# yumingj/Text2Human

Hardware: AMD Instinct MI355X
Metric: 512x256 images/sec (sample_from_parsing) (higher is better)
Workload: dtype f16 hi plane + e4m3 cross-term planes, f32 accumulate (hidden err 4e-5, tokens exact); exact-f32: exact_fp32_path

## Files before the change

### text2human_amd/csrc/gemm_split.hip

```cpp
#include <hip/hip_ext.h>
#include <stdlib.h>

#include <type_traits>

#include "common.h"

namespace {

typedef t2h_f16x8 f16x8;
typedef unsigned int u32x4 __attribute__((ext_vector_type(4)));

constexpr int SP_TILE_B = T2H_SPLIT_TILE_B;
constexpr int SP_LDS_ROW = 144;
constexpr int SP_PIECES = 8;

__device__ __forceinline__ void gload16_async(u32x4& dst, const char* ptr) {
#ifdef T2H_SDBG_NOGLOAD
  asm volatile("" : "=v"(dst) : "v"(ptr));
#else
  asm volatile("global_load_dwordx4 %0, %1, off" : "=v"(dst) : "v"(ptr) : "memory");
#endif
}
__device__ __forceinline__ void gload16_async(u32x4& dst, unsigned voff, const char* sbase) {
#ifdef T2H_SDBG_NOGLOAD
  asm volatile("" : "=v"(dst) : "v"(voff), "s"(sbase));
#else
  asm volatile("global_load_dwordx4 %0, %1, %2" : "=v"(dst) : "v"(voff), "s"(sbase) : "memory");
#endif
}
template <int N>
__device__ __forceinline__ void wait_vmcnt16(u32x4& v) {
  asm volatile("s_waitcnt vmcnt(%1)" : "+v"(v) : "n"(N));
}

__device__ __forceinline__ float erf_rational(float x) {
  x = fminf(fmaxf(x, -4.0f), 4.0f);
  const float x2 = x * x;
  float p = -2.72614225801306e-10f;
  p = fmaf(p, x2, 2.77068142495902e-08f);
  p = fmaf(p, x2, -2.10102402082508e-06f);
  p = fmaf(p, x2, -5.69250639462346e-05f);
  p = fmaf(p, x2, -7.34990630326855e-04f);
  p = fmaf(p, x2, -2.95459980854025e-03f);
  p = fmaf(p, x2, -1.60960333262415e-02f);
  float q = -1.45660718464996e-05f;
  q = fmaf(q, x2, -2.13374055278905e-04f);
  q = fmaf(q, x2, -1.68282697438203e-03f);
  q = fmaf(q, x2, -7.37332916720468e-03f);
  q = fmaf(q, x2, -1.42647390514189e-02f);
  return x * p * __builtin_amdgcn_rcpf(q);
}

__device__ __forceinline__ float gelu_erf_s(float v) {
  return 0.5f * v * (1.0f + erf_rational(v * 0.70710678118654752440f));
}

typedef float f32x2 __attribute__((ext_vector_type(2)));
__device__ __forceinline__ f32x2 gelu_erf_2(f32x2 v) {
  f32x2 x = v * 0.70710678118654752440f;
  x[0] = fminf(fmaxf(x[0], -4.0f), 4.0f);
  x[1] = fminf(fmaxf(x[1], -4.0f), 4.0f);
  const f32x2 x2 = x * x;
  auto fma2 = [](f32x2 a, f32x2 b, float c) { return __builtin_elementwise_fma(a, b, f32x2{c, c}); };
  f32x2 p = {-2.72614225801306e-10f, -2.72614225801306e-10f};
  p = fma2(p, x2, 2.77068142495902e-08f);
  p = fma2(p, x2, -2.10102402082508e-06f);
  p = fma2(p, x2, -5.69250639462346e-05f);
  p = fma2(p, x2, -7.34990630326855e-04f);
  p = fma2(p, x2, -2.95459980854025e-03f);
  p = fma2(p, x2, -1.60960333262415e-02f);
  f32x2 q = {-1.45660718464996e-05f, -1.45660718464996e-05f};
  q = fma2(q, x2, -2.13374055278905e-04f);
  q = fma2(q, x2, -1.68282697438203e-03f);
  q = fma2(q, x2, -7.37332916720468e-03f);
  q = fma2(q, x2, -1.42647390514189e-02f);
  const f32x2 rq = {__builtin_amdgcn_rcpf(q[0]), __builtin_amdgcn_rcpf(q[1])};
  const f32x2 e = x * p * rq;
  return (v * 0.5f) * (e + 1.0f);
}
__device__ __forceinline__ f32x4 gelu_erf_v(f32x4 v) {
  const f32x2 a = gelu_erf_2(f32x2{v[0], v[1]}), b = gelu_erf_2(f32x2{v[2], v[3]});
  return f32x4{a[0], a[1], b[0], b[1]};
}

#ifdef T2H_SDBG_HOTLOAD
#define LM0 0
#define LN0 0
#else
#define LM0 m0
#define LN0 n0
#endif

#define G1_MARK(i)                                                                                      \
  do {                                                                                                  \
    if (probe != nullptr && threadIdx.x == 0) {                                                         \
      probe[(int64_t)blockIdx.x * 16 + (i)] = (long long)__builtin_amdgcn_s_memrealtime();              \
      probe[(int64_t)blockIdx.x * 16 + 8 + (i)] = (long long)__builtin_amdgcn_s_memtime();              \
    }                                                                                                   \
  } while (0)

typedef int i32x8 __attribute__((ext_vector_type(8)));
__device__ __forceinline__ f32x16 x8_cross(const f16x8& a0, const f16x8& a1, const f16x8& b0, const f16x8& b1, const f32x16& c) {
  union { f16x8 h[2]; i32x8 v; } ua, ub;
  ua.h[0] = a0;
  ua.h[1] = a1;
  ub.h[0] = b0;
  ub.h[1] = b1;
  return __builtin_amdgcn_mfma_scale_f32_32x32x64_f8f6f4(ua.v, ub.v, c, 0, 0, 0, 0x7f7f7f7f, 0, 0x7f7f7f7f);
}

template <int BM, int BN, int WARPS_M, int WARPS_N, int KS, int PP, int FMT = 0>
__global__ __launch_bounds__(64 * WARPS_M * WARPS_N * KS) void gemm_split_kernel(const t2h_gemm_split_args p, int* const ovf, long long* const probe) {
  constexpr int NT = 64 * WARPS_M * WARPS_N;
  constexpr int NWG = WARPS_M * WARPS_N;
  constexpr int WM = BM / WARPS_M, WN = BN / WARPS_N;
  constexpr int TM = WM / 32, TN = WN / 32;
  static_assert(TM >= 1 && TN >= 1, "wave tile must hold a 32x32 MFMA tile");
  constexpr int PIECES = (BM + BN) * SP_PIECES;
  constexpr int L = (PIECES + NT - 1) / NT;
  constexpr int NMMA = 2 * 3 * TM * TN;
  constexpr int BUF_B = (BM + BN) * SP_LDS_ROW;
  constexpr int O_LD = WN + 4;
  constexpr int OT_LD = WM + 4;
  constexpr int OW = WM * O_LD > WN * OT_LD ? WM * O_LD : WN * OT_LD;
  constexpr int EPI_B = OW * 4 * NWG * KS;
  constexpr int TILE_IMG_B = (BM + BN) * SP_TILE_B;
  constexpr int MAIN_B = PP == 2 ? 3 * TILE_IMG_B : 2 * BUF_B * KS;
  constexpr int SMEM_B = MAIN_B > EPI_B ? MAIN_B : EPI_B;

  __shared__ __attribute__((aligned(16))) char smem[SMEM_B];

  G1_MARK(0);
  const int kg = KS == 1 ? 0 : (int)threadIdx.x / NT;
  const int tid = threadIdx.x - kg * NT;
  const int lane = tid & 63, wave = tid >> 6;
  char* const gsm = smem + kg * (2 * BUF_B);
  const int l31 = lane & 31, hh = lane >> 5;
  const int wm0 = (wave / WARPS_N) * WM, wn0 = (wave % WARPS_N) * WN;
  const int nbx = (p.N + BN - 1) / BN, nby = (p.M + BM - 1) / BM;
  const int ksid = (PP == 2 && p.ksplit > 1) ? __builtin_amdgcn_readfirstlane((int)blockIdx.x / (nbx * nby)) : 0;
  int m0, n0;
  {
    const int total = nbx * nby, b = (int)blockIdx.x - ksid * (nbx * nby);
    const int xcd = b & 7, slot = b >> 3, q = total >> 3, r = total & 7;
    const int lin = (xcd < r ? xcd * (q + 1) : r * (q + 1) + (xcd - r) * q) + slot;
    int mt = lin / nbx, nt = lin - mt * nbx;
    if (r == 0 && q <= 32 && nbx >= 16 && (nbx & 1) == 0 && (nby & 3) == 0 && q == (nby >> 2) * (nbx >> 1)) {
      const int hbx = nbx >> 1;
      const int sr = slot / hbx;
      mt = (xcd >> 1) * (nby >> 2) + sr;
      nt = (xcd & 1) * hbx + (slot - sr * hbx);
    }
    m0 = mt * BM;
    n0 = nt * BN;
  }
  const int nk_row = p.K / (32 * KS);
  const int nk = (PP == 2 && p.ksplit > 1) ? nk_row >> (p.ksplit >> 1) : nk_row;
  const int last = nk - 1;
  const int64_t row_b = (int64_t)nk_row * (SP_TILE_B * KS);
  const int64_t k_base = (int64_t)__builtin_amdgcn_readfirstlane(ksid * nk) * SP_TILE_B;
  constexpr int K_STEP_B = SP_TILE_B * KS;

  f32x16 acc[2][TM][TN];
#pragma unroll
  for (int c = 0; c < 2; ++c)
#pragma unroll
    for (int i = 0; i < TM; ++i)
#pragma unroll
      for (int j = 0; j < TN; ++j)
#pragma unroll
        for (int r = 0; r < 16; ++r) acc[c][i][j][r] = 0.f;

  if constexpr (PP == 2) {
    static_assert(KS == 1 && NWG == 8 && (BM + BN) % 64 == 0, "ping-pong DMA: 8 waves, whole 8-row groups per wave");
    constexpr int NL = (BM + BN) / 64;
    const int grp = __builtin_amdgcn_readfirstlane(wave >> 2);
    auto pp_barrier = [] {
      __builtin_amdgcn_sched_barrier(0);
#ifndef T2H_SDBG_NOBAR
      __builtin_amdgcn_s_barrier();
#endif
      __builtin_amdgcn_sched_barrier(0);
    };
    const unsigned lds0 = (unsigned)(uintptr_t)smem;
    unsigned goff[NL];
#pragma unroll
    for (int i = 0; i < NL; ++i) {
      const int g = wave + 8 * i;
      const int r = g * 8 + (lane >> 3), pc = (lane & 7) ^ ((r >> 1) & 7);
      const bool isA = r < BM;
      const int grow = isA ? min(LM0 + r, p.M - 1) : min(LN0 + r - BM, p.N - 1);
      goff[i] = (unsigned)grow * (unsigned)row_b + pc * 16;
    }
    static_assert(BM % 64 == 0, "an 8-row group belongs to one operand");
    const unsigned wdst = __builtin_amdgcn_readfirstlane(lds0 + wave * 1024);
    auto dma = [&](int kt, unsigned buf_off) {
      if (kt > last) return;
      const int64_t k0 = (int64_t)kt * SP_TILE_B + k_base;
      const char* const baseA = reinterpret_cast<const char*>(p.A) + k0;
      const char* const baseB = reinterpret_cast<const char*>(p.B) + k0;
#pragma unroll
      for (int i = 0; i < NL; ++i) {
#ifndef T2H_SDBG_NOGLOAD
        unsigned keep;
#ifdef T2H_SDBG_HALFDMA
        if (i & 1) continue;
#endif
        const char* const base = i < BM / 64 ? baseA : baseB;
        const unsigned dst_i = wdst + buf_off + i * 8192;
#ifndef T2H_DMA_POLICY
#define T2H_DMA_POLICY " nt"
#endif
        asm volatile("s_mov_b32 %0, m0\n\ts_mov_b32 m0, %3\n\ts_nop 0\n\tglobal_load_lds_dwordx4 %1, %2" T2H_DMA_POLICY "\n\ts_mov_b32 m0, %0"
                     : "=&s"(keep)
                     : "v"(goff[i]), "s"(base), "s"(dst_i)
                     : "memory");
#endif
      }
    };
    auto wait_landed = [&](bool younger_in_flight) {
      __builtin_amdgcn_sched_barrier(0);
      if (younger_in_flight) asm volatile("s_waitcnt vmcnt(%0)" ::"n"(NL) : "memory");
      else asm volatile("s_waitcnt vmcnt(0)" ::: "memory");
      __builtin_amdgcn_sched_barrier(0);
    };
    const int swz = (l31 >> 1) & 7;
    int offA[4], offB[4];
#pragma unroll
    for (int c2 = 0; c2 < 4; ++c2) {
      const int pcs = ((c2 * 2 + hh) ^ swz) * 16;
      offA[c2] = (wm0 + l31) * 128 + pcs;
      offB[c2] = (BM + wn0 + l31) * 128 + pcs;
      if (FMT == 1 && c2 >= 2) {
        offA[c2] = (wm0 + l31) * 128 + ((4 + 2 * hh + (c2 - 2)) ^ swz) * 16;
        offB[c2] = (BM + wn0 + l31) * 128 + ((4 + 2 * (1 - hh) + (c2 - 2)) ^ swz) * 16;
      }
    }
    constexpr int PA[3] = {1, 0, 0};
    constexpr int PB[3] = {0, 1, 0};
    constexpr int PC[3] = {1, 1, 0};
    dma(0, 0);
    dma(1, TILE_IMG_B);
    wait_landed(nk > 1);
    pp_barrier();
    G1_MARK(1);
    if (grp == 1) pp_barrier();
    unsigned b_cur = 0, b_nxt = TILE_IMG_B, b_free = 2 * TILE_IMG_B;
    for (int kt = 0; kt < nk; ++kt) {
      const char* img = smem + b_cur;
      f16x8 af[2][TM][2], bfr[2][TN][2];
#ifdef T2H_SDBG_DMAFIRST
      dma(kt + 2, b_free);
      __builtin_amdgcn_sched_barrier(0);
#endif
#pragma unroll
      for (int u = 0; u < 2; ++u) {
#pragma unroll
        for (int ti = 0; ti < TM; ++ti)
#pragma unroll
          for (int pl = 0; pl < 2; ++pl)
#ifdef T2H_SDBG_NOFRAG
            asm volatile("" : "=v"(af[u][ti][pl]) : "v"(img));
#else
            af[u][ti][pl] = *reinterpret_cast<const f16x8*>(img + ti * 32 * 128 + offA[pl * 2 + u]);
#endif
#pragma unroll
        for (int tj = 0; tj < TN; ++tj)
#pragma unroll
          for (int pl = 0; pl < 2; ++pl)
#ifdef T2H_SDBG_NOFRAG
            asm volatile("" : "=v"(bfr[u][tj][pl]) : "v"(img));
#else
            bfr[u][tj][pl] = *reinterpret_cast<const f16x8*>(img + tj * 32 * 128 + offB[pl * 2 + u]);
#endif
      }
      __builtin_amdgcn_sched_barrier(0);
#ifndef T2H_SDBG_DMAFIRST
      dma(kt + 2, b_free);
#endif
      if (grp == 1) wait_landed(kt + 2 < nk);
      asm volatile("s_waitcnt lgkmcnt(0)" ::: "memory");
      pp_barrier();
      if constexpr (FMT == 1) {
#pragma unroll
        for (int ti = 0; ti < TM; ++ti)
#pragma unroll
          for (int tj = 0; tj < TN; ++tj) {
            acc[0][ti][tj] = __builtin_amdgcn_mfma_f32_32x32x16_f16(af[0][ti][0], bfr[0][tj][0], acc[0][ti][tj], 0, 0, 0);
            acc[1][ti][tj] = x8_cross(af[0][ti][1], af[1][ti][1], bfr[0][tj][1], bfr[1][tj][1], acc[1][ti][tj]);
          }
#pragma unroll
        for (int ti = 0; ti < TM; ++ti)
#pragma unroll
          for (int tj = 0; tj < TN; ++tj)
            acc[0][ti][tj] = __builtin_amdgcn_mfma_f32_32x32x16_f16(af[1][ti][0], bfr[1][tj][0], acc[0][ti][tj], 0, 0, 0);
      } else {
#pragma unroll
      for (int u = 0; u < 2; ++u)
#pragma unroll
        for (int t = 0; t < 3; ++t)
#pragma unroll
          for (int ti = 0; ti < TM; ++ti)
#pragma unroll
            for (int tj = 0; tj < TN; ++tj) {
#ifdef T2H_SDBG_NOMMA
              asm volatile("" : "+v"(acc[PC[t]][ti][tj]) : "v"(af[u][ti][PA[t]]), "v"(bfr[u][tj][PB[t]]));
#else
              acc[PC[t]][ti][tj] = __builtin_amdgcn_mfma_f32_32x32x16_f16(af[u][ti][PA[t]], bfr[u][tj][PB[t]],
                                                                           acc[PC[t]][ti][tj], 0, 0, 0);
#endif
            }
      }
      if (grp == 0) wait_landed(kt + 2 < nk);
      pp_barrier();
      const unsigned t = b_cur;
      b_cur = b_nxt;
      b_nxt = b_free;
      b_free = t;
    }
    if (grp == 0) pp_barrier();
    asm volatile("s_waitcnt vmcnt(0)" ::: "memory");
    __syncthreads();
  } else {
  static_assert(PIECES % NT == 0 && (BM * SP_PIECES) % NT == 0, "whole rounds of pieces, each of one operand");
  constexpr int LA = BM * SP_PIECES / NT;
  unsigned src[L];
  int dst[L];
#pragma unroll
  for (int i = 0; i < L; ++i) {
    const int q = tid + NT * i;
    const int row = q / SP_PIECES, pc = q - row * SP_PIECES;
    const bool isA = i < LA;
    const int grow = isA ? min(LM0 + row, p.M - 1) : min(LN0 + row - BM, p.N - 1);
    src[i] = (unsigned)grow * (unsigned)row_b + kg * SP_TILE_B + pc * 16;
    dst[i] = row * SP_LDS_ROW + pc * 16;
  }
  const char* const gA = reinterpret_cast<const char*>(p.A);
  const char* const gB = reinterpret_cast<const char*>(p.B);
  u32x4 rg[2][L];
#ifdef T2H_SDBG_NOPUT
  auto put = [&](int i, const u32x4& r, int buf) { asm volatile("" ::"v"(r), "v"(dst[i] + buf)); };
#else
  auto put = [&](int i, const u32x4& r, int buf) { *reinterpret_cast<u32x4*>(gsm + buf * BUF_B + dst[i]) = r; };
#endif
  auto issue = [&](auto setc, int kt) {
    constexpr int S = decltype(setc)::value;
    const int64_t k0 = (int64_t)min(kt, last) * K_STEP_B;
#pragma unroll
    for (int i = 0; i < L; ++i) gload16_async(rg[S][i], src[i], (i < LA ? gA : gB) + k0);
  };

  using set0 = std::integral_constant<int, 0>;
  using set1 = std::integral_constant<int, 1>;
  issue(set0{}, 0);
  issue(set1{}, 1);
#pragma unroll
  for (int i = 0; i < L; ++i) {
    wait_vmcnt16<L>(rg[0][i]);
    put(i, rg[0][i], 0);
  }
  __builtin_amdgcn_sched_barrier(0);
  issue(set0{}, 2);
  __syncthreads();
  G1_MARK(1);

  constexpr int PA[3] = {1, 0, 0};
  constexpr int PB[3] = {0, 1, 0};
  constexpr int PC[3] = {1, 1, 0};

  constexpr int NMMA_F = FMT == 1 ? 3 * TM * TN : NMMA;
  auto step = [&](int kt, auto setc) {
    constexpr int S = decltype(setc)::value;
    const int buf = kt & 1;
    const int64_t kn = (int64_t)min(kt + 3, last) * K_STEP_B;
    const char* Ab = gsm + buf * BUF_B + (wm0 + l31) * SP_LDS_ROW + hh * 16;
    const char* Bb = gsm + buf * BUF_B + (BM + wn0 + l31) * SP_LDS_ROW + hh * 16;
    int mma = 0;
    auto pinned = [&]() {
      ++mma;
#pragma unroll
      for (int q = 0; q < L; ++q) {
        const int at0 = (2 * L <= NMMA_F) ? NMMA_F - 2 * (L - q) + 1 : (NMMA_F * (q + 1)) / L;
        const int at = at0 < 1 ? 1 : at0;
        if (at != mma) continue;
        __builtin_amdgcn_sched_barrier(0);
        wait_vmcnt16<2 * L - 1>(rg[S][q]);
        put(q, rg[S][q], buf ^ 1);
        __builtin_amdgcn_sched_barrier(0);
        gload16_async(rg[S][q], src[q], (q < LA ? gA : gB) + kn);
        __builtin_amdgcn_sched_barrier(0);
      }
    };
    if constexpr (FMT == 1) {
      f16x8 ah[2][TM], a8[2][TM], bh[2][TN], b8[2][TN];
#pragma unroll
      for (int j = 0; j < 2; ++j) {
#pragma unroll
        for (int ti = 0; ti < TM; ++ti) {
          ah[j][ti] = *reinterpret_cast<const f16x8*>(Ab + ti * 32 * SP_LDS_ROW + j * 32);
          a8[j][ti] = *reinterpret_cast<const f16x8*>(Ab + ti * 32 * SP_LDS_ROW + 64 + hh * 16 + j * 16);
        }
#pragma unroll
        for (int tj = 0; tj < TN; ++tj) {
          bh[j][tj] = *reinterpret_cast<const f16x8*>(Bb + tj * 32 * SP_LDS_ROW + j * 32);
          b8[j][tj] = *reinterpret_cast<const f16x8*>(Bb + tj * 32 * SP_LDS_ROW + 96 - 48 * hh + j * 16);
        }
      }
#pragma unroll
      for (int ti = 0; ti < TM; ++ti)
#pragma unroll
        for (int tj = 0; tj < TN; ++tj) {
          acc[0][ti][tj] = __builtin_amdgcn_mfma_f32_32x32x16_f16(ah[0][ti], bh[0][tj], acc[0][ti][tj], 0, 0, 0);
          pinned();
          acc[1][ti][tj] = x8_cross(a8[0][ti], a8[1][ti], b8[0][tj], b8[1][tj], acc[1][ti][tj]);
          pinned();
        }
#pragma unroll
      for (int ti = 0; ti < TM; ++ti)
#pragma unroll
        for (int tj = 0; tj < TN; ++tj) {
          acc[0][ti][tj] = __builtin_amdgcn_mfma_f32_32x32x16_f16(ah[1][ti], bh[1][tj], acc[0][ti][tj], 0, 0, 0);
          pinned();
        }
    } else {
#pragma unroll
    for (int u = 0; u < 2; ++u) {
      f16x8 af[TM][2], bfr[TN][2];
#pragma unroll
      for (int ti = 0; ti < TM; ++ti)
#pragma unroll
        for (int pl = 0; pl < 2; ++pl)
#ifdef T2H_SDBG_NOFRAG
          asm volatile("" : "=v"(af[ti][pl]) : "v"(Ab));
#else
          af[ti][pl] = *reinterpret_cast<const f16x8*>(Ab + ti * 32 * SP_LDS_ROW + pl * 64 + u * 32);
#endif
#pragma unroll
      for (int tj = 0; tj < TN; ++tj)
#pragma unroll
        for (int pl = 0; pl < 2; ++pl)
#ifdef T2H_SDBG_NOFRAG
          asm volatile("" : "=v"(bfr[tj][pl]) : "v"(Bb));
#else
          bfr[tj][pl] = *reinterpret_cast<const f16x8*>(Bb + tj * 32 * SP_LDS_ROW + pl * 64 + u * 32);
#endif
#pragma unroll
      for (int t = 0; t < 3; ++t) {
#pragma unroll
        for (int ti = 0; ti < TM; ++ti)
#pragma unroll
          for (int tj = 0; tj < TN; ++tj) {
#ifdef T2H_SDBG_NOMMA
            asm volatile("" : "+v"(acc[PC[t]][ti][tj]) : "v"(af[ti][PA[t]]), "v"(bfr[tj][PB[t]]));
#else
            acc[PC[t]][ti][tj] = __builtin_amdgcn_mfma_f32_32x32x16_f16(af[ti][PA[t]], bfr[tj][PB[t]],
                                                                         acc[PC[t]][ti][tj], 0, 0, 0);
#endif
            pinned();
          }
      }
    }
    }
    __syncthreads();
  };
  for (int kt = 0; kt < nk; kt += 2) {
    step(kt, set1{});
    if (kt + 1 < nk) step(kt + 1, set0{});
  }
#pragma unroll
  for (int S = 0; S < 2; ++S)
#pragma unroll
    for (int i = 0; i < L; ++i) wait_vmcnt16<0>(rg[S][i]);
  }
// ... 77 lines not shown
  __syncthreads();
  constexpr int CPR = WN / 8;
  constexpr int NCH = WM * CPR / 64 / KS;
  static_assert(NCH >= 1 && NCH * 64 * KS == WM * CPR, "epilogue chunking");
#pragma unroll
  for (int it = 0; it < NCH; ++it) {
    const int c = lane + 64 * (it + kg * NCH);
    const int rl = c / CPR, c8 = (c - rl * CPR) * 8;
    const int row = m0 + wm0 + rl, col = n0 + wn0 + c8;
    const bool valid = row < p.M && col < p.N && !(MIXED && some_v && col >= p.vt_col0);
    if (!valid) continue;
    f32x4 va = *reinterpret_cast<const f32x4*>(Ot + rl * O_LD + c8);
    f32x4 vb = *reinterpret_cast<const f32x4*>(Ot + rl * O_LD + c8 + 4);
    if (KS == 2) {
      va += *reinterpret_cast<const f32x4*>(Ot + NWG * OW + rl * O_LD + c8);
      vb += *reinterpret_cast<const f32x4*>(Ot + NWG * OW + rl * O_LD + c8 + 4);
    }
    if (p.epi_act == 1) {
      va = gelu_erf_v(va);
      vb = gelu_erf_v(vb);
    } else if (p.epi_act == 2) {
#pragma unroll
      for (int e = 0; e < 4; ++e) {
        va[e] = fmaxf(va[e], 0.f);
        vb[e] = fmaxf(vb[e], 0.f);
      }
    }
    if (p.residual && ksid == 0) {
      va += *reinterpret_cast<const f32x4*>(p.residual + (int64_t)row * p.ldr + col);
      vb += *reinterpret_cast<const f32x4*>(p.residual + (int64_t)row * p.ldr + col + 4);
    }
    if (p.C) {
      float* const Cs = p.C + (int64_t)ksid * p.M * p.ldc;
      *reinterpret_cast<f32x4*>(Cs + (int64_t)row * p.ldc + col) = va;
      *reinterpret_cast<f32x4*>(Cs + (int64_t)row * p.ldc + col + 4) = vb;
    }
    if (p.C_split) {
      if (p.out_fmt == 1) t2h_store_x8_8<1>(p.C_split, row, p.N, col, va, vb, p.out_scale, ovf);
      else t2h_store_split8(p.C_split, row, p.N, col, va, vb, ovf);
    }
  }
  G1_MARK(3);
#ifdef T2H_GEMM_TIMING
  asm volatile("s_waitcnt vmcnt(0)" ::: "memory");
  G1_MARK(4);
#endif
}

constexpr int SKINNY_WAVES = 8;
typedef int i32x8s __attribute__((ext_vector_type(8)));
template <int FMT>
__global__ __launch_bounds__(64 * SKINNY_WAVES) void gemm_split_skinny_kernel(const t2h_gemm_split_args p, int* const ovf) {
  __shared__ __attribute__((aligned(16))) float red[SKINNY_WAVES][16 * 16];
  const int wave = threadIdx.x >> 6, lane = threadIdx.x & 63;
  const int r = lane & 15, kg = lane >> 4;
  const int n0 = blockIdx.x * 16, m0 = blockIdx.y * 16;
  const int nk = p.K / 32;
  const int64_t row_b = (int64_t)nk * SP_TILE_B;
  const char* ap = reinterpret_cast<const char*>(p.A) + (int64_t)min(m0 + r, p.M - 1) * row_b + kg * 16;
  const char* bp = reinterpret_cast<const char*>(p.B) + (int64_t)min(n0 + r, p.N - 1) * row_b + kg * 16;
  f32x4 acc = {0.f, 0.f, 0.f, 0.f}, acc_lo = acc;
  if constexpr (FMT == 1) {
    const char* a8 = reinterpret_cast<const char*>(p.A) + (int64_t)min(m0 + r, p.M - 1) * row_b + 64 + (kg & 1) * 32;
    const char* b8 = reinterpret_cast<const char*>(p.B) + (int64_t)min(n0 + r, p.N - 1) * row_b + 64 + (1 - (kg & 1)) * 32;
    const int npair = (nk + 1) / 2;
#pragma unroll 2
    for (int t2 = wave; t2 < npair; t2 += SKINNY_WAVES) {
      const int t0 = 2 * t2, tg = t0 + (kg >> 1);
      const bool have = tg < nk;
      union { f16x8 h[2]; i32x8s v; } ua, ub;
      const f16x8 zero = {0, 0, 0, 0, 0, 0, 0, 0};
      ua.h[0] = have ? *reinterpret_cast<const f16x8*>(a8 + (int64_t)tg * SP_TILE_B) : zero;
      ua.h[1] = have ? *reinterpret_cast<const f16x8*>(a8 + (int64_t)tg * SP_TILE_B + 16) : zero;
      ub.h[0] = have ? *reinterpret_cast<const f16x8*>(b8 + (int64_t)tg * SP_TILE_B) : zero;
      ub.h[1] = have ? *reinterpret_cast<const f16x8*>(b8 + (int64_t)tg * SP_TILE_B + 16) : zero;
      acc_lo = __builtin_amdgcn_mfma_scale_f32_16x16x128_f8f6f4(ua.v, ub.v, acc_lo, 0, 0, 0, 0x7f7f7f7f, 0, 0x7f7f7f7f);
      acc = __builtin_amdgcn_mfma_f32_16x16x32_f16(*reinterpret_cast<const f16x8*>(ap + (int64_t)t0 * SP_TILE_B),
                                                   *reinterpret_cast<const f16x8*>(bp + (int64_t)t0 * SP_TILE_B), acc, 0, 0, 0);
      if (t0 + 1 < nk)
        acc = __builtin_amdgcn_mfma_f32_16x16x32_f16(*reinterpret_cast<const f16x8*>(ap + (int64_t)(t0 + 1) * SP_TILE_B),
                                                     *reinterpret_cast<const f16x8*>(bp + (int64_t)(t0 + 1) * SP_TILE_B), acc, 0, 0, 0);
    }
  } else {
#pragma unroll 4
  for (int t = wave; t < nk; t += SKINNY_WAVES) {
    const f16x8 ah = *reinterpret_cast<const f16x8*>(ap + (int64_t)t * SP_TILE_B);
    const f16x8 al = *reinterpret_cast<const f16x8*>(ap + (int64_t)t * SP_TILE_B + 64);
    const f16x8 bh = *reinterpret_cast<const f16x8*>(bp + (int64_t)t * SP_TILE_B);
    const f16x8 bl = *reinterpret_cast<const f16x8*>(bp + (int64_t)t * SP_TILE_B + 64);
    acc_lo = __builtin_amdgcn_mfma_f32_16x16x32_f16(al, bh, acc_lo, 0, 0, 0);
    acc_lo = __builtin_amdgcn_mfma_f32_16x16x32_f16(ah, bl, acc_lo, 0, 0, 0);
    acc = __builtin_amdgcn_mfma_f32_16x16x32_f16(ah, bh, acc, 0, 0, 0);
  }
  }
  const float lo_mul = FMT == 1 ? p.lo_mul : T2H_SPLIT_LO_INV;
#pragma unroll
  for (int e = 0; e < 4; ++e) red[wave][(4 * kg + e) * 16 + r] = fmaf(acc_lo[e], lo_mul, acc[e]);
  __syncthreads();
  if (wave != 0) return;
  const int rl = lane >> 2, c4 = (lane & 3) * 4;
  const int row = m0 + rl, col = n0 + c4;
  if (row >= p.M || col >= p.N) return;
  f32x4 v = *reinterpret_cast<const f32x4*>(&red[0][rl * 16 + c4]);
#pragma unroll
  for (int w = 1; w < SKINNY_WAVES; ++w) v += *reinterpret_cast<const f32x4*>(&red[w][rl * 16 + c4]);
  if (p.bias) v += *reinterpret_cast<const f32x4*>(p.bias + col);
  if (p.epi_act == 1) v = gelu_erf_v(v);
  else if (p.epi_act == 2)
#pragma unroll
    for (int e = 0; e < 4; ++e) v[e] = fmaxf(v[e], 0.f);
  if (p.residual) v += *reinterpret_cast<const f32x4*>(p.residual + (int64_t)row * p.ldr + col);
  if (p.C) *reinterpret_cast<f32x4*>(p.C + (int64_t)row * p.ldc + col) = v;
  if (p.C_split) {
    if (p.out_fmt == 1) t2h_store_x8_4(p.C_split, row, p.N, col, v, p.out_scale, ovf);
    else t2h_store_split4(p.C_split, row, p.N, col, v, ovf);
  }
}

__global__ void split_rows_kernel(const float* __restrict__ x, int ldx, uint16_t* __restrict__ out, int64_t total,
                                  int C, int* ovf) {
  const int64_t i = (int64_t)blockIdx.x * blockDim.x + threadIdx.x;
  if (i >= total) return;
  const int q = C >> 2;
  const int64_t row = i / q;
  const int c0 = (int)(i - row * q) * 4;
  t2h_store_split4(out, row, C, c0, *reinterpret_cast<const f32x4*>(x + row * ldx + c0), ovf);
}

__global__ void split_rows_x8_kernel(const float* __restrict__ x, int ldx, uint16_t* __restrict__ out, int64_t total,
                                     int C, float scale, int* ovf) {
  const int64_t i = (int64_t)blockIdx.x * blockDim.x + threadIdx.x;
  if (i >= total) return;
  const int q = C >> 2;
  const int64_t row = i / q;
  const int c0 = (int)(i - row * q) * 4;
  t2h_store_x8_4(out, row, C, c0, *reinterpret_cast<const f32x4*>(x + row * ldx + c0), scale, ovf);
}

thread_local hipEvent_t g_time_start = nullptr, g_time_stop = nullptr;
thread_local long long* g_probe = nullptr;

template <typename K, typename... Args>
void launch_maybe_timed(K kernel, dim3 grid, dim3 block, hipStream_t s, Args... args) {
  if (g_time_start && g_time_stop) {
    hipExtLaunchKernelGGL(kernel, grid, block, 0, s, g_time_start, g_time_stop, 0, args...);
    g_time_start = g_time_stop = nullptr;
  } else {
    hipLaunchKernelGGL(kernel, grid, block, 0, s, args...);
  }
}

template <int BM, int BN, int WARPS_M, int WARPS_N, int KS = 1, int PP = 0, int FMT = 0>
int launch_split(const t2h_gemm_split_args& a, hipStream_t s) {
  T2H_REQUIRE(a.K % (32 * KS) == 0, "t2h_gemm_split_f32: this tile config needs K %% %d == 0", 32 * KS);
  if (a.Vt)
    T2H_REQUIRE(a.vt_col0 % (BN % 128 ? 32 : BN) == 0, "t2h_gemm_split_f32: vt_col0=%d must be a multiple of %d for this tile",
                a.vt_col0, BN % 128 ? 32 : BN);
  T2H_REQUIRE((int64_t)(a.M > a.N ? a.M : a.N) * a.K * 4 < (int64_t(1) << 31),
              "t2h_gemm_split_f32: operands are addressed with 32-bit byte offsets (each must span < 2 GiB)");
  const int ks = a.ksplit > 1 ? a.ksplit : 1;
  if (ks > 1)
    T2H_REQUIRE(PP == 2 && a.K % (32 * ks) == 0 && a.C && !a.C_split && !a.Vt && a.epi_act == 0,
                "t2h_gemm_split_f32: ksplit=%d needs a ping-pong tile configuration (8, 10, 11), K %% %d == 0, an fp32 output "
                "of ksplit * M rows and no activation / split-row / Vt output", ks, 32 * ks);
  dim3 grid(((a.N + BN - 1) / BN) * ((a.M + BM - 1) / BM) * ks);
  int* ovf = a.overflow_flag;
  launch_maybe_timed(gemm_split_kernel<BM, BN, WARPS_M, WARPS_N, KS, PP, FMT>, grid, dim3(64 * WARPS_M * WARPS_N * KS), s, a,
                     ovf, g_probe);
  T2H_CHECK_LAUNCH("t2h_gemm_split_f32");
  return T2H_OK;
}

thread_local int g_force_split_cfg = -1;

}

extern "C" int t2h_gemm_split_probe_next_launch(void* dev_int64_buf) {
  g_probe = static_cast<long long*>(dev_int64_buf);
  return T2H_OK;
}

extern "C" int t2h_gemm_split_time_next_launch(void* start_event, void* stop_event) {
  g_time_start = static_cast<hipEvent_t>(start_event);
  g_time_stop = static_cast<hipEvent_t>(stop_event);
  return T2H_OK;
}

extern "C" int t2h_gemm_split_force_config(int cfg) {
  const int old = g_force_split_cfg;
  g_force_split_cfg = cfg;
  return old;
}

static int pick_split_cfg(const t2h_gemm_split_args& a) {
  int cfg = g_force_split_cfg;
  if (cfg < 0) {
    const int64_t tiles64 = (int64_t)((a.M + 127) / 128) * ((a.N + 63) / 64);
    const int64_t tiles128 = (int64_t)((a.M + 127) / 128) * ((a.N + 127) / 128);
    const int64_t tiles256 = (int64_t)((a.M + 127) / 128) * ((a.N + 255) / 256);
    const int64_t tiles_big = (a.M % 256 == 0 && a.N % 128 == 0) ? (int64_t)(a.M / 256) * (a.N / 128) : 0;
    const int64_t cus = 256;
    if (a.M <= 64) cfg = 2;
    else if (tiles_big >= cus * 3 / 4) {
      cfg = 8;
      if (a.M % 128 == 0 && a.N % 192 == 0 && (a.Vt == nullptr || a.vt_col0 % 32 == 0)) {
        const int64_t t192 = (int64_t)(a.M / 128) * (a.N / 192);
        if (((t192 + cus - 1) / cus) * (128 * 192) < ((tiles_big + cus - 1) / cus) * (256 * 128)) cfg = 10;
      }
    } else if (tiles128 >= 4 * cus) cfg = 1;
    else if (tiles64 <= cus && a.K % 64 == 0 && a.K >= 256) cfg = 6;
    else cfg = 0;
  }
  const bool skinny_ok = a.N % 16 == 0 && !a.Vt && (a.bias == nullptr || t2h_aligned16(a.bias));
  if (g_force_split_cfg < 0 && a.M <= 64 && skinny_ok) cfg = 9;
  return cfg;
}

extern "C" int t2h_gemm_split_tile_config(const t2h_gemm_split_args* args) {
  T2H_REQUIRE(args != nullptr && args->M > 0 && args->N > 0 && args->K > 0, "t2h_gemm_split_tile_config: bad arguments");
  return pick_split_cfg(*args);
}

extern "C" int t2h_gemm_split_f32(const t2h_gemm_split_args* args, void* stream) {
  struct Disarm {
    ~Disarm() {
      g_time_start = g_time_stop = nullptr;
      g_probe = nullptr;
    }
  } disarm_on_exit;
  T2H_REQUIRE(args != nullptr, "t2h_gemm_split_f32: args is NULL");
  const t2h_gemm_split_args a = *args;
  T2H_REQUIRE(a.A && a.B && (a.C || a.C_split || a.Vt), "t2h_gemm_split_f32: NULL operand");
  T2H_REQUIRE(a.M > 0 && a.N > 0 && a.K > 0 && a.K % 32 == 0, "t2h_gemm_split_f32: bad shape M=%d N=%d K=%d",
              a.M, a.N, a.K);
  T2H_REQUIRE(t2h_aligned16(a.A) && t2h_aligned16(a.B), "t2h_gemm_split_f32: operands must be 16-byte aligned");
  T2H_REQUIRE(a.N % 8 == 0 && (!a.C || (a.ldc % 4 == 0 && t2h_aligned16(a.C))) &&
                  (!a.residual || (a.ldr % 4 == 0 && t2h_aligned16(a.residual))),
              "t2h_gemm_split_f32: N must be a multiple of 8, ldc / ldr of 4, C / residual 16-byte aligned");
  if (a.C_split) T2H_REQUIRE(a.N % 32 == 0, "t2h_gemm_split_f32: split output needs N %% 32 == 0");
  T2H_REQUIRE(a.overflow_flag != nullptr || (!a.C_split && !a.Vt),
              "t2h_gemm_split_f32: overflow_flag is NULL (needed with C_split / Vt outputs)");
  if (a.Vt)
    T2H_REQUIRE(a.vt_hd > 0 && a.vt_T > 0 && a.vt_T % 128 == 0 && a.M % a.vt_T == 0 && a.vt_col0 >= 0 &&
                    a.vt_col0 < a.N && (a.N - a.vt_col0) % a.vt_hd == 0 && a.epi_act == 0 && !a.residual,
                "t2h_gemm_split_f32: bad Vt routing (col0=%d T=%d hd=%d M=%d N=%d)", a.vt_col0, a.vt_T, a.vt_hd,
                a.M, a.N);
  T2H_REQUIRE((a.fmt == 0 || a.fmt == 1) && (a.out_fmt == 0 || a.out_fmt == 1), "t2h_gemm_split_f32: fmt / out_fmt must be 0 or 1");
  T2H_REQUIRE(a.ksplit >= 0 && a.ksplit <= 4 && a.ksplit != 3, "t2h_gemm_split_f32: ksplit must be 0 / 1 (off), 2 or 4");
  if (a.ksplit > 1)
    T2H_REQUIRE(a.fmt == 1 && (pick_split_cfg(a) == 8 || pick_split_cfg(a) == 10 || pick_split_cfg(a) == 11),
                "t2h_gemm_split_f32: ksplit needs x8 operands on a ping-pong tile configuration (force 8, 10 or 11)");
  hipStream_t s = static_cast<hipStream_t>(stream);
  t2h_gemm_split_args ax = a;
  if (ax.lo_mul == 0.f) ax.lo_mul = T2H_SPLIT_LO_INV;
  if (ax.out_scale == 0.f) ax.out_scale = 1.0f;
  const int cfg = pick_split_cfg(a);
  if (cfg == 9) {
    const bool skinny_ok = a.N % 16 == 0 && !a.Vt && (a.bias == nullptr || t2h_aligned16(a.bias));
    T2H_REQUIRE(skinny_ok, "t2h_gemm_split_f32: the few-rows kernel needs N %% 16 == 0 and no Vt routing");
    int* ovf = a.overflow_flag;
    if (a.fmt == 1)
      launch_maybe_timed(gemm_split_skinny_kernel<1>, dim3(a.N / 16, (a.M + 15) / 16), dim3(64 * SKINNY_WAVES), s, ax, ovf);
    else
      launch_maybe_timed(gemm_split_skinny_kernel<0>, dim3(a.N / 16, (a.M + 15) / 16), dim3(64 * SKINNY_WAVES), s, ax, ovf);
    T2H_CHECK_LAUNCH("t2h_gemm_split_f32");
    return T2H_OK;
  }
  if (a.fmt == 1) {
    switch (cfg) {
      case 2: return launch_split<64, 64, 2, 2, 1, 0, 1>(ax, s);
      case 6: return launch_split<128, 64, 2, 2, 2, 0, 1>(ax, s);
      case 8: return launch_split<256, 128, 4, 2, 1, 2, 1>(ax, s);
      case 10: return launch_split<128, 192, 4, 2, 1, 2, 1>(ax, s);
      case 11: return launch_split<128, 128, 4, 2, 1, 2, 1>(ax, s);
      case 0: return launch_split<128, 64, 2, 2, 1, 0, 1>(ax, s);
      default:
        t2h_set_error("t2h_gemm_split_f32: tile configuration %d is not built for x8 operands (0, 2, 6, 8, 9, 10, 11)", cfg);
        return T2H_ERR_INVALID;
    }
  }
  switch (cfg) {
    case 1: return launch_split<128, 128, 4, 2>(ax, s);
    case 2: return launch_split<64, 64, 2, 2>(ax, s);
    case 3: return launch_split<128, 64, 4, 2>(ax, s);
    case 5: return launch_split<128, 256, 4, 2>(ax, s);
    case 6: return launch_split<128, 64, 2, 2, 2>(ax, s);
    case 8: return launch_split<256, 128, 4, 2, 1, 2>(ax, s);
    case 10: return launch_split<128, 192, 4, 2, 1, 2>(ax, s);
    default: return launch_split<128, 64, 2, 2>(ax, s);
  }
}

extern "C" int t2h_split_rows_x8_f32(const float* x, int32_t ldx, uint16_t* out, int64_t rows, int32_t C, float scale,
                                     int32_t* overflow_flag, void* stream) {
  T2H_REQUIRE(x && out && rows > 0 && C > 0 && C % 32 == 0 && ldx % 4 == 0 && scale > 0.f, "t2h_split_rows_x8_f32: bad arguments");
  T2H_REQUIRE(overflow_flag != nullptr, "t2h_split_rows_x8_f32: overflow_flag is NULL");
  const int64_t total = rows * (C / 4);
  hipLaunchKernelGGL(split_rows_x8_kernel, dim3((unsigned)((total + 255) / 256)), dim3(256), 0,
                     static_cast<hipStream_t>(stream), x, ldx, out, total, C, scale, overflow_flag);
  T2H_CHECK_LAUNCH("t2h_split_rows_x8_f32");
  return T2H_OK;
}

extern "C" int t2h_split_rows_f32(const float* x, int32_t ldx, uint16_t* out, int64_t rows, int32_t C,
                                  int32_t* overflow_flag, void* stream) {
  T2H_REQUIRE(x && out && rows > 0 && C > 0 && C % 32 == 0 && ldx % 4 == 0, "t2h_split_rows_f32: bad arguments");
  const int64_t total = rows * (C / 4);
  int* ovf = overflow_flag;
  T2H_REQUIRE(ovf != nullptr, "t2h_split_rows_f32: overflow_flag is NULL");
  hipLaunchKernelGGL(split_rows_kernel, dim3((unsigned)((total + 255) / 256)), dim3(256), 0,
                     static_cast<hipStream_t>(stream), x, ldx, out, total, C, ovf);
  T2H_CHECK_LAUNCH("t2h_split_rows_f32");
  return T2H_OK;
}
```

### text2human_amd/ops.py

```python
import ctypes
import os

import torch

from . import _lib
from ._lib import GemmArgs, check

ACT_NONE, ACT_GELU, ACT_RELU = 0, 1, 2
PRO_NONE, PRO_SWISH = 0, 1


def _p(t):
    return ctypes.c_void_p(t.data_ptr()) if t is not None else ctypes.c_void_p(0)


def _stream():
    return ctypes.c_void_p(torch.cuda.current_stream().cuda_stream)


_ovf_slots = {}


def _ovf_slot():
    dev = torch.cuda.current_device()
    key = (dev, torch.cuda.current_stream().cuda_stream)
    slot = _ovf_slots.get(key)
    if slot is None:
        if torch.cuda.is_current_stream_capturing():
            raise _lib.T2HError('the overflow flag of this stream must exist before a capture begins: call '
                                'ops.split_overflow(reset=True) on the stream first')
        slot = _ovf_slots[key] = (torch.zeros(1, dtype=torch.int32, device=f'cuda:{dev}'),
                                  torch.zeros(1, dtype=torch.int32).pin_memory())
    return slot


def overflow_flag():
    return ctypes.c_void_p(_ovf_slot()[0].data_ptr())


def release_overflow_flag(stream=None):
    st = stream if stream is not None else torch.cuda.current_stream()
    _ovf_slots.pop((torch.cuda.current_device(), st.cuda_stream), None)


def _chk_f32(*ts):
    for t in ts:
        if t is None:
            continue
        if t.dtype != torch.float32 or not t.is_cuda:
            raise TypeError(f'expected CUDA float32 tensor, got {t.dtype} on {t.device}')


def _chk_i64(*ts):
    for t in ts:
        if t.dtype != torch.int64 or not t.is_cuda or not t.is_contiguous():
            raise TypeError('expected contiguous CUDA int64 tensor')


def _rows(t):
    if t.dim() != 2 or t.stride(1) != 1:
        raise ValueError(f'need a 2-D tensor with unit inner stride, got {tuple(t.shape)} {t.stride()}')
    return t.stride(0)


GEMM_CFG_NAMES = ['64x64x32', '128x32x32', '128x64x32', '128x128x32', '128x64x64', '128x128x64',
                  '128x64x32w8', '128x64x64w8', '128x128x64w8']


def gemm_force_config(cfg):
    return _lib.load().t2h_gemm_force_config(int(cfg))


_prof = None


def gemm_profile_start(every=1):
    global _prof
    _prof = dict(every=max(1, int(every)), count=0, recs=[])


def gemm_profile_active():
    return _prof is not None


SPLIT_CFG_NAMES = {0: '128x64', 1: '128x128', 2: '64x64', 3: '128x64, 8 waves', 5: '128x256', 6: '128x64, 2 K groups',
                   8: '256x128, ping-pong LDS-DMA', 9: 'few rows (16x16 per workgroup, K over 8 waves)',
                   10: '128x192, ping-pong LDS-DMA', 11: '128x128, ping-pong LDS-DMA'}


def _probe_clock(buf):
    t = buf.view(-1, 16).cpu()
    t = t[(t[:, 1] != 0) & (t[:, 2] != 0)].double()
    if t.shape[0] == 0:
        return None
    us = (t[:, 2] - t[:, 1]) * 0.01
    ghz = (t[:, 10] - t[:, 9]) / (us * 1e3)
    return float(us.median()), float(ghz.median())


def gemm_profile_stop():
    global _prof
    p, _prof = _prof, None
    if not p:
        return {}
    torch.cuda.synchronize()
    out = {}

    def add(r, flops, e0, e1, kind, probe):
        if kind == 'stream':
            r['n_stream'] += 1
            r['ms_stream'] += e0.elapsed_time(e1)
            r['flops_stream'] += flops
            return
        r['kernel_timed'] = r['kernel_timed'] or kind == 'kernel'
        r['n'] += 1
        r['ms'] += e0.elapsed_time(e1)
        r['flops'] += flops
        if probe is not None:
            r['n_probe'] += 1
            r['loop_us'] += probe[0]
            r['loop_ghz'] += probe[1]

    blank = lambda label: dict(kernel=label, n=0, ms=0.0, flops=0.0, n_stream=0, ms_stream=0.0, flops_stream=0.0,
                               kernel_timed=False, n_probe=0, loop_us=0.0, loop_ghz=0.0)
    for rec in p['recs']:
        label, flops, e0, e1 = rec[:4]
        kind = rec[4] if len(rec) > 4 else None
        cfg = rec[5] if len(rec) > 5 else None
        probe = _probe_clock(rec[6]) if len(rec) > 6 and rec[6] is not None else None
        r = out.setdefault(label, blank(label))
        add(r, flops, e0, e1, kind, probe)
        if cfg is not None:
            name = f'gemm_split_kernel<{SPLIT_CFG_NAMES.get(cfg, cfg)}>'
            add(r.setdefault('by_cfg', {}).setdefault(name, blank(name)), flops, e0, e1, kind, probe)
    return out


def _launch_gemm(g, what):
    lib = _lib.load()
    if _prof is not None:
        _prof['count'] += 1
        if _prof['count'] % _prof['every'] == 0:
            cfg = lib.t2h_gemm_tile_config(ctypes.byref(g))
            label = (f"gemm_kernel<{GEMM_CFG_NAMES[cfg]},amode={g.a_mode},"
                     f"pro={int(bool(g.pro_scale))},btrans={g.b_trans}>")
            flops = 2.0 * g.M * g.N * g.K * max(1, g.batch)
            e0, e1 = torch.cuda.Event(enable_timing=True), torch.cuda.Event(enable_timing=True)
            e0.record()
            check(lib.t2h_gemm_f32(ctypes.byref(g), _stream()), what)
            e1.record()
            _prof['recs'].append((label, flops, e0, e1))
            return
    check(lib.t2h_gemm_f32(ctypes.byref(g), _stream()), what)


def gemm(a, w, out=None, bias=None, residual=None, act=ACT_NONE, alpha=1.0, pro=None,
         b_trans=False):
    _chk_f32(a, w, out, bias, residual)
    M, K = a.shape
    N = w.shape[1] if b_trans else w.shape[0]
    assert (w.shape[0] if b_trans else w.shape[1]) == K, (a.shape, w.shape)
    if out is None:
        out = torch.empty((M, N), device=a.device, dtype=torch.float32)
    g = GemmArgs()
    g.A, g.B, g.C = a.data_ptr(), w.data_ptr(), out.data_ptr()
    g.bias = bias.data_ptr() if bias is not None else None
    g.residual = residual.data_ptr() if residual is not None else None
    g.M, g.N, g.K = M, N, K
    g.lda, g.ldb, g.ldc = _rows(a), _rows(w), _rows(out)
    g.ldr = _rows(residual) if residual is not None else 0
    g.a_mode, g.b_trans, g.epi_act, g.alpha = 0, int(b_trans), act, alpha
    if pro is not None:
        sc, sh, rows, pact = pro
        _chk_f32(sc, sh)
        g.pro_scale, g.pro_shift = sc.data_ptr(), sh.data_ptr()
        g.pro_rows, g.pro_ld, g.pro_act = rows, sc.shape[1], pact
    g.batch = 1
    _launch_gemm(g, 't2h_gemm_f32')
    return out


def _launch_conv_split(g, flops):
    lib = _lib.load()
    if _prof is not None:
        _prof['count'] += 1
        if _prof['count'] % _prof['every'] == 0:
            e0, e1 = torch.cuda.Event(enable_timing=True), torch.cuda.Event(enable_timing=True)
            e0.record()
            check(lib.t2h_conv_split_f32(ctypes.byref(g), _stream()), 't2h_conv_split_f32')
            e1.record()
            _prof['recs'].append(('conv_split_kernel<2xfp16>', flops, e0, e1))
            return
    check(lib.t2h_conv_split_f32(ctypes.byref(g), _stream()), 't2h_conv_split_f32')


def conv_split_ok(n_pix_per_img, mode='same', act=ACT_NONE):
    return mode in ('same', 'up') and n_pix_per_img % 128 == 0 and act in (ACT_NONE, ACT_RELU)


def gn_apply_split(x, scale=None, shift=None, rows_per_img=0, act=PRO_NONE, out=None):
    _chk_f32(x, scale, shift)
    rows, C = x.shape
    if out is None:
        out = split_rows_empty(rows, C, x.device)
    check(_lib.load().t2h_gn_apply_split_f32(_p(x), _rows(x), _p(scale), _p(shift),
                                             scale.shape[1] if scale is not None else 0, _p(out), rows,
                                             rows_per_img, C, act, overflow_flag(), _stream()), 't2h_gn_apply_split_f32')
    return out


def conv_split(xs, w_split, n_img, hin, win, cin, cout, taps=9, out=None, bias=None, residual=None,
               act=ACT_NONE, mode='same', res_pre=False, gn_stats=False):
    _chk_f32(out, bias, residual)
    assert mode in ('same', 'up') and taps in (1, 9)
    ups = 1 if mode == 'up' else 0
    hout, wout = hin << ups, win << ups
    M = n_img * hout * wout
    assert xs.numel() == n_img * hin * win * cin * 2 and w_split.numel() == cout * taps * cin * 2, \
        (tuple(xs.shape), tuple(w_split.shape), n_img, hin, win, cin, cout, taps)
    if out is None:
        out = torch.empty((M, cout), device=xs.device, dtype=torch.float32)
    g = GemmArgs()
    g.A, g.B, g.C = xs.data_ptr(), w_split.data_ptr(), out.data_ptr()
    g.bias = bias.data_ptr() if bias is not None else None
    g.residual = residual.data_ptr() if residual is not None else None
    g.M, g.N, g.K = M, cout, taps * cin
    g.lda, g.ldb, g.ldc = 0, 0, _rows(out)
    g.ldr = _rows(residual) if residual is not None else 0
    g.a_mode, g.epi_act, g.alpha, g.res_pre = 1, act, 1.0, int(res_pre)
    g.Hin, g.Win, g.Cin, g.Hout, g.Wout = hin, win, cin, hout, wout
    g.stride, g.pad, g.ups, g.batch = 1, (1 if taps == 9 else 0), ups, 1
    part = None
    if gn_stats:
        part = torch.empty((n_img, hout * wout // 128, 2, cout), device=xs.device, dtype=torch.float64)
        g.gn_part_out = part.data_ptr()
    _launch_conv_split(g, 2.0 * M * cout * taps * cin)
    if part is not None:
        out._t2h_gn_part = part
    return out

# ... 713 lines not shown
```

Baseline: 12.18.

## Add 128x64 two-K-group LDS-DMA triple-buffered GEMM tile configuration

Adds a new PP==3 path to the split GEMM kernel: a 128x64 tile with two K groups of two waves each, loading operands into a swizzled three-slot LDS ring via global_load_lds DMA. MFMA issue is interleaved with the DMA and fragment reads for the next step. The config is registered as case 12 for both operand formats. Nothing in the visible code makes pick_split_cfg choose 12, so it seems reachable only through a forced config, and it requires K to be a multiple of 128.

```diff
diff --git a/text2human_amd/csrc/gemm_split.hip b/text2human_amd/csrc/gemm_split.hip
--- a/text2human_amd/csrc/gemm_split.hip
+++ b/text2human_amd/csrc/gemm_split.hip
@@ -125,7 +125,7 @@
   constexpr int OW = WM * O_LD > WN * OT_LD ? WM * O_LD : WN * OT_LD;
   constexpr int EPI_B = OW * 4 * NWG * KS;
   constexpr int TILE_IMG_B = (BM + BN) * SP_TILE_B;
-  constexpr int MAIN_B = PP == 2 ? 3 * TILE_IMG_B : 2 * BUF_B * KS;
+  constexpr int MAIN_B = PP == 2 ? 3 * TILE_IMG_B : PP == 3 ? 3 * TILE_IMG_B * KS : 2 * BUF_B * KS;
   constexpr int SMEM_B = MAIN_B > EPI_B ? MAIN_B : EPI_B;
 
   __shared__ __attribute__((aligned(16))) char smem[SMEM_B];
@@ -319,6 +319,141 @@
       b_free = t;
     }
     if (grp == 0) pp_barrier();
+    asm volatile("s_waitcnt vmcnt(0)" ::: "memory");
+    __syncthreads();
+  } else if constexpr (PP == 3) {
+    static_assert(KS == 2 && NWG == 2 && WARPS_N == 1 && BM % 16 == 0 && BN % 16 == 0, "W4: 2 K groups x 2 waves");
+    constexpr int NL = (BM + BN) / 16;
+    constexpr int NR = 4 * (TM + TN);
+    const int kgs = __builtin_amdgcn_readfirstlane(kg);
+    const unsigned lds0 = (unsigned)(uintptr_t)smem;
+    unsigned goff[NL];
+#pragma unroll
+    for (int i = 0; i < NL; ++i) {
+      const int g = wave + 2 * i;
+      const int r = g * 8 + (lane >> 3), pc = (lane & 7) ^ ((r >> 1) & 7);
+      const int grow = i < BM / 16 ? min(LM0 + r, p.M - 1) : min(LN0 + r - BM, p.N - 1);
+      goff[i] = (unsigned)grow * (unsigned)row_b + pc * 16;
+    }
+    const unsigned wdst = __builtin_amdgcn_readfirstlane(lds0 + kgs * (3 * TILE_IMG_B) + wave * 1024);
+    auto dma = [&](int kt, int i0, int i1) {
+      const int64_t k0 = (int64_t)(2 * kt + kgs) * SP_TILE_B;
+      const char* const baseA = reinterpret_cast<const char*>(p.A) + k0;
+      const char* const baseB = reinterpret_cast<const char*>(p.B) + k0;
+      const unsigned buf_off = (unsigned)(kt % 3) * TILE_IMG_B;
+#pragma unroll
+      for (int i = i0; i < i1; ++i) {
+        unsigned keep;
+        const char* const base = i < BM / 16 ? baseA : baseB;
+        const unsigned dst_i = wdst + buf_off + i * 2048;
+        asm volatile("s_mov_b32 %0, m0\n\ts_mov_b32 m0, %3\n\ts_nop 0\n\tglobal_load_lds_dwordx4 %1, %2" T2H_DMA_POLICY "\n\ts_mov_b32 m0, %0"
+                     : "=&s"(keep)
+                     : "v"(goff[i]), "s"(base), "s"(dst_i)
+                     : "memory");
+      }
+    };
+    const int swz = (l31 >> 1) & 7;
+    int offA[4], offB[4];
+#pragma unroll
+    for (int c2 = 0; c2 < 4; ++c2) {
+      const int pcs = ((c2 * 2 + hh) ^ swz) * 16;
+      offA[c2] = (wm0 + l31) * 128 + pcs;
+      offB[c2] = (BM + wn0 + l31) * 128 + pcs;
+      if (FMT == 1 && c2 >= 2) {
+        offA[c2] = (wm0 + l31) * 128 + ((4 + 2 * hh + (c2 - 2)) ^ swz) * 16;
+        offB[c2] = (BM + wn0 + l31) * 128 + ((4 + 2 * (1 - hh) + (c2 - 2)) ^ swz) * 16;
+      }
+    }
+    const char* const ring = smem + kgs * (3 * TILE_IMG_B);
+    f16x8 af[2][2][TM][2], bfr[2][2][TN][2];
+    constexpr int RU[4] = {0, 0, 1, 1};
+    constexpr int RP[4] = {0, 1, FMT == 1 ? 1 : 0, FMT == 1 ? 0 : 1};
+    auto frag = [&](auto setc, int n, const char* img) {
+      constexpr int S = decltype(setc)::value;
+      const int blk = n / (TM + TN), e = n - blk * (TM + TN);
+      const int u = RU[blk], pl = RP[blk];
+      if (e < TM) af[S][u][e][pl] = *reinterpret_cast<const f16x8*>(img + e * 32 * 128 + offA[pl * 2 + u]);
+      else bfr[S][u][e - TM][pl] = *reinterpret_cast<const f16x8*>(img + (e - TM) * 32 * 128 + offB[pl * 2 + u]);
+    };
+    constexpr int PA[3] = {1, 0, 0};
+    constexpr int PB[3] = {0, 1, 0};
+    constexpr int PC[3] = {1, 1, 0};
+    constexpr int NM = FMT == 1 ? 3 * TM * TN : 6 * TM * TN;
+    auto mma = [&](auto setc, int m) {
+      constexpr int S = decltype(setc)::value;
+      if constexpr (FMT == 1) {
+        if (m < 2 * TM * TN) {
+          const int b = m >> 1, ti = b / TN, tj = b - ti * TN;
+          if ((m & 1) == 0)
+            acc[0][ti][tj] = __builtin_amdgcn_mfma_f32_32x32x16_f16(af[S][0][ti][0], bfr[S][0][tj][0], acc[0][ti][tj], 0, 0, 0);
+          else
+            acc[1][ti][tj] = x8_cross(af[S][0][ti][1], af[S][1][ti][1], bfr[S][0][tj][1], bfr[S][1][tj][1], acc[1][ti][tj]);
+        } else {
+          const int b = m - 2 * TM * TN, ti = b / TN, tj = b - ti * TN;
+          acc[0][ti][tj] = __builtin_amdgcn_mfma_f32_32x32x16_f16(af[S][1][ti][0], bfr[S][1][tj][0], acc[0][ti][tj], 0, 0, 0);
+        }
+      } else {
+        const int u = m / (3 * TM * TN), r = m - u * (3 * TM * TN), t = r / (TM * TN), b = r - t * (TM * TN);
+        const int ti = b / TN, tj = b - ti * TN;
+        acc[PC[t]][ti][tj] = __builtin_amdgcn_mfma_f32_32x32x16_f16(af[S][u][ti][PA[t]], bfr[S][u][tj][PB[t]],
+                                                                     acc[PC[t]][ti][tj], 0, 0, 0);
+      }
+    };
+    constexpr int MB = NM / 3;
+    auto step = [&](int kt, auto setc, auto nextc, auto dmac, auto waitc) {
+      constexpr bool DMA = decltype(dmac)::value;
+      constexpr int WAITN = decltype(waitc)::value;
+#pragma unroll
+      for (int m = 0; m < MB; ++m) mma(setc, m);
+      __builtin_amdgcn_sched_barrier(0);
+      asm volatile("s_waitcnt lgkmcnt(0)" ::: "memory");
+      if constexpr (WAITN == 0) asm volatile("s_waitcnt vmcnt(0)" ::: "memory");
+      else asm volatile("s_waitcnt vmcnt(%0)" ::"n"(WAITN) : "memory");
+      __builtin_amdgcn_sched_barrier(0);
+      __builtin_amdgcn_s_barrier();
+      __builtin_amdgcn_sched_barrier(0);
+      const char* const img = ring + ((kt + 1) % 3) * TILE_IMG_B;
+#pragma unroll
+      for (int m = MB; m < NM; ++m) {
+        mma(setc, m);
+        __builtin_amdgcn_sched_barrier(0);
+        const int j = m - MB, J = NM - MB;
+        if constexpr (DMA) dma(kt + 3, NL * j / J, NL * (j + 1) / J);
+#pragma unroll
+        for (int n = NR * j / J; n < NR * (j + 1) / J; ++n) frag(nextc, n, img);
+        __builtin_amdgcn_sched_barrier(0);
+      }
+    };
+    using set0 = std::integral_constant<int, 0>;
+    using set1 = std::integral_constant<int, 1>;
+    using dma1 = std::integral_constant<bool, true>;
+    using dma0 = std::integral_constant<bool, false>;
+    using waitNL = std::integral_constant<int, NL>;
+    using wait0 = std::integral_constant<int, 0>;
+    dma(0, 0, NL);
+    dma(1, 0, NL);
+    if (nk > 2) dma(2, 0, NL);
+    constexpr int NL2 = 2 * NL;
+    if (nk > 2) asm volatile("s_waitcnt vmcnt(%0)" ::"n"(NL2) : "memory");
+    else asm volatile("s_waitcnt vmcnt(%0)" ::"n"(NL) : "memory");
+    __builtin_amdgcn_sched_barrier(0);
+    __builtin_amdgcn_s_barrier();
+    __builtin_amdgcn_sched_barrier(0);
+#pragma unroll
+    for (int n = 0; n < NR; ++n) frag(set0{}, n, ring);
+    G1_MARK(1);
+    int kt = 0;
+    for (; kt + 6 <= nk; kt += 2) {
+      step(kt, set0{}, set1{}, dma1{}, waitNL{});
+      step(kt + 1, set1{}, set0{}, dma1{}, waitNL{});
+    }
+    if (kt + 4 == nk) {
+      step(kt, set0{}, set1{}, dma1{}, waitNL{});
+      step(kt + 1, set1{}, set0{}, dma0{}, waitNL{});
+      kt += 2;
+    }
+    step(kt, set0{}, set1{}, dma0{}, wait0{});
+    step(kt + 1, set1{}, set0{}, dma0{}, wait0{});
     asm volatile("s_waitcnt vmcnt(0)" ::: "memory");
     __syncthreads();
   } else {
@@ -702,7 +837,8 @@
 
 template <int BM, int BN, int WARPS_M, int WARPS_N, int KS = 1, int PP = 0, int FMT = 0>
 int launch_split(const t2h_gemm_split_args& a, hipStream_t s) {
-  T2H_REQUIRE(a.K % (32 * KS) == 0, "t2h_gemm_split_f32: this tile config needs K %% %d == 0", 32 * KS);
+  T2H_REQUIRE(a.K % (PP == 3 ? 128 : 32 * KS) == 0, "t2h_gemm_split_f32: this tile config needs K %% %d == 0",
+              PP == 3 ? 128 : 32 * KS);
   if (a.Vt)
     T2H_REQUIRE(a.vt_col0 % (BN % 128 ? 32 : BN) == 0, "t2h_gemm_split_f32: vt_col0=%d must be a multiple of %d for this tile",
                 a.vt_col0, BN % 128 ? 32 : BN);
@@ -820,12 +956,13 @@
     switch (cfg) {
       case 2: return launch_split<64, 64, 2, 2, 1, 0, 1>(ax, s);
       case 6: return launch_split<128, 64, 2, 2, 2, 0, 1>(ax, s);
+      case 12: return launch_split<128, 64, 2, 1, 2, 3, 1>(ax, s);
       case 8: return launch_split<256, 128, 4, 2, 1, 2, 1>(ax, s);
       case 10: return launch_split<128, 192, 4, 2, 1, 2, 1>(ax, s);
       case 11: return launch_split<128, 128, 4, 2, 1, 2, 1>(ax, s);
       case 0: return launch_split<128, 64, 2, 2, 1, 0, 1>(ax, s);
       default:
-        t2h_set_error("t2h_gemm_split_f32: tile configuration %d is not built for x8 operands (0, 2, 6, 8, 9, 10, 11)", cfg);
+        t2h_set_error("t2h_gemm_split_f32: tile configuration %d is not built for x8 operands (0, 2, 6, 8, 9, 10, 11, 12)", cfg);
         return T2H_ERR_INVALID;
     }
   }
@@ -835,6 +972,7 @@
     case 3: return launch_split<128, 64, 4, 2>(ax, s);
     case 5: return launch_split<128, 256, 4, 2>(ax, s);
     case 6: return launch_split<128, 64, 2, 2, 2>(ax, s);
+    case 12: return launch_split<128, 64, 2, 1, 2, 3>(ax, s);
     case 8: return launch_split<256, 128, 4, 2, 1, 2>(ax, s);
     case 10: return launch_split<128, 192, 4, 2, 1, 2>(ax, s);
     default: return launch_split<128, 64, 2, 2>(ax, s);
diff --git a/text2human_amd/ops.py b/text2human_amd/ops.py
--- a/text2human_amd/ops.py
+++ b/text2human_amd/ops.py
@@ -85,7 +85,8 @@
 
 SPLIT_CFG_NAMES = {0: '128x64', 1: '128x128', 2: '64x64', 3: '128x64, 8 waves', 5: '128x256', 6: '128x64, 2 K groups',
                    8: '256x128, ping-pong LDS-DMA', 9: 'few rows (16x16 per workgroup, K over 8 waves)',
-                   10: '128x192, ping-pong LDS-DMA', 11: '128x128, ping-pong LDS-DMA'}
+                   10: '128x192, ping-pong LDS-DMA', 11: '128x128, ping-pong LDS-DMA',
+                   12: '128x64, 2 K groups x 2 waves, LDS-DMA'}
 
 
 def _probe_clock(buf):
```

Result: slower. 12.02, median of 6 (-1.3%).
